# hongsukchoi/Pose2Mesh_RELEASE

Hardware: AMD Instinct MI355X
Metric: SMPL meshes/sec fwd+bwd at batch 256 (higher is better)
Workload: dtype f32 (emulated on the BF16 matrix pipe: every operand as 3 exact bf16 slices = 24-bit significands, 6 slice products per fp32 product, fp32 accumulate)

## Files before the change

pose2mesh_release_amd/csrc/basis.hip:

```cpp
#include <cstdlib>

#include "p2m_common.h"

namespace p2m {

constexpr int ROWS_PER_BLOCK = 4;

static int basis_spb() { return 8; }

static bool basis_tiled() {
  static int v = [] { const char* e = getenv("P2M_BASIS_TILED"); return e ? atoi(e) : 1; }();
  return v != 0;
}

__device__ __forceinline__ int xcd_swizzle(int bid, int nb) {
  return (nb & 7) == 0 ? (bid & 7) * (nb >> 3) + (bid >> 3) : bid;
}

__device__ __forceinline__ void fma4(float4& acc, float s, const float4& x) {
  acc.x = fmaf(s, x.x, acc.x); acc.y = fmaf(s, x.y, acc.y);
  acc.z = fmaf(s, x.z, acc.z); acc.w = fmaf(s, x.w, acc.w);
}

template <int LPR>
// ... 287 lines not shown
    const int u = q % U, sl = q / U, b = b0 + sl;
    if (b < B) {
      const float* src = G + ((long)b * V + pl.ucol[u0 + u]) * NC;
#pragma unroll
      for (int c = 0; c < NC; c++) xs[sl][u][c] = src[c];
    }
  }
  __syncthreads();
  const int i = t % TILE_RMAX, sl = t / TILE_RMAX, b = b0 + sl;
  if (i >= R || b >= B) return;
  const long ridx = (long)b * V + real_ids[r0 + i];
  float t1[NC], t2[NC];
#pragma unroll
  for (int c = 0; c < NC; c++) t1[c] = t2[c] = 0.f;
  for (int j = rowoff[i]; j < rowoff[i + 1]; j++) {
    const float4 en = ents[j];
    const float* q = xs[sl][__float_as_int(en.z)];
#pragma unroll
    for (int c = 0; c < NC; c++) {
      t1[c] = fmaf(en.x, q[c], t1[c]);
      t2[c] = fmaf(en.y, q[c], t2[c]);
    }
  }
  float* e = E + ridx * lde;
#pragma unroll
  for (int c = 0; c < NC; c++) {
    e[c] = G[ridx * NC + c];
    e[NC + c] = t1[c];
    e[2 * NC + c] = t2[c];
  }
  for (int c = 3 * NC; c < lde; c++) e[c] = 0.f;
}

}

using namespace p2m;

static int combine_small_launch(p2m_graph_t gh, const float* P, int32_t ldp, int32_t nc, const float* bias, float* Y,
                                int32_t B, int real_only, const int32_t* out_index, int32_t out_rows, float scale,
                                void* stream) {
  const Graph& g = *reinterpret_cast<const Graph*>(gh);
  const int* ids = real_only ? g.real_ids : nullptr;
  const int nset = real_only ? g.n_real : g.V;
  const long tot = (long)B * nset;
  if (tot == 0) return P2M_OK;
  hipStream_t s = (hipStream_t)stream;
  int skip_real = 0;
  const TilePlan& pl = g.plan[0];
  if (pl.ntiles > 0 && basis_tiled() && nc == 3) {
    hipLaunchKernelGGL(k_combine_small_tile<3>, dim3(pl.ntiles * cdiv(B, SMALL_SPB)), dim3(256), 0, s, pl, g.real_ids, g.V,
                       P, ldp, bias, Y, B, out_index, out_rows, scale);
    if (real_only) return check_launch("cheb_combine_small(tiled)");
    skip_real = 1;
  }
#define P2M_COMBINE(NCv) hipLaunchKernelGGL(k_combine_small<NCv>, dim3(cdiv(tot, 256)), dim3(256), 0, s, g, P, ldp, bias, \
                                            Y, B, ids, nset, out_index, out_rows, scale, skip_real)
  switch (nc) {
    case 1: P2M_COMBINE(1); break;
    case 2: P2M_COMBINE(2); break;
    case 3: P2M_COMBINE(3); break;
    case 4: P2M_COMBINE(4); break;
    default: set_error("p2m_cheb_combine_small: nc must be 1..4 (got %d)", nc); return P2M_ERR_INVALID;
  }
#undef P2M_COMBINE
  return check_launch("cheb_combine_small");
}

extern "C" int p2m_cheb_combine_small(p2m_graph_t gh, const float* P, int32_t ldp, int32_t nc, const float* bias,
                                      float* Y, int32_t B, void* stream) {
  P2M_CHECK_ARG(gh && P && Y && ldp >= 3 * nc, "null pointer or ldp < 3*nc");
  if (B <= 0) return P2M_OK;
  return combine_small_launch(gh, P, ldp, nc, bias, Y, B, 0, nullptr, 0, 1.f, stream);
}

extern "C" int p2m_cheb_combine_small_real(p2m_graph_t gh, const float* P, int32_t ldp, int32_t nc, const float* bias,
                                           float* Y, int32_t B, const int32_t* out_index, int32_t out_rows,
                                           float scale, void* stream) {
  P2M_CHECK_ARG(gh && P && Y && ldp >= 3 * nc, "null pointer or ldp < 3*nc");
  P2M_CHECK_ARG(out_index == nullptr || out_rows > 0, "out_rows must be positive with out_index");
  if (B <= 0) return P2M_OK;
  return combine_small_launch(gh, P, ldp, nc, bias, Y, B, 1, out_index, out_rows, scale, stream);
}

extern "C" int p2m_cheb_expand_small(p2m_graph_t gh, const float* G, int32_t nc, float* E, int32_t lde, int32_t B,
                                     void* stream) {
  P2M_CHECK_ARG(gh && G && E && lde >= 3 * nc, "null pointer or lde < 3*nc");
  if (B <= 0) return P2M_OK;
  const Graph& g = *reinterpret_cast<const Graph*>(gh);
  const long tot = (long)B * g.V;
  hipStream_t s = (hipStream_t)stream;
  int skip_real = 0;
  const TilePlan& pl = g.plan[0];
  if (pl.ntiles > 0 && basis_tiled() && nc == 3) {
    hipLaunchKernelGGL(k_expand_small_tile<3>, dim3(pl.ntiles * cdiv(B, SMALL_SPB)), dim3(256), 0, s, pl, g.real_ids, g.V,
                       G, E, lde, B);
    skip_real = 1;
  }
  switch (nc) {
    case 1: hipLaunchKernelGGL(k_expand_small<1>, dim3(cdiv(tot, 256)), dim3(256), 0, s, g, G, E, lde, B, skip_real); break;
    case 2: hipLaunchKernelGGL(k_expand_small<2>, dim3(cdiv(tot, 256)), dim3(256), 0, s, g, G, E, lde, B, skip_real); break;
    case 3: hipLaunchKernelGGL(k_expand_small<3>, dim3(cdiv(tot, 256)), dim3(256), 0, s, g, G, E, lde, B, skip_real); break;
    case 4: hipLaunchKernelGGL(k_expand_small<4>, dim3(cdiv(tot, 256)), dim3(256), 0, s, g, G, E, lde, B, skip_real); break;
    default: set_error("p2m_cheb_expand_small: nc must be 1..4 (got %d)", nc); return P2M_ERR_INVALID;
  }
  return check_launch("cheb_expand_small");
}


namespace p2m {
typedef float f32x4v __attribute__((ext_vector_type(4)));

template <int LPR>
__global__ __launch_bounds__(512, 2) void k_basis_tile(TilePlan pl, const float* __restrict__ X,
                                                        float* __restrict__ T1, float* __restrict__ T2, int B, int F,
                                                        long x_rows, int nset, int spb,
                                                        const float* __restrict__ in_scale = nullptr,
                                                        const float* __restrict__ in_shift = nullptr) {
  constexpr int NT = 512;
  constexpr int FB = LPR * 4;
  constexpr int RPI = NT / LPR;
  constexpr int NPF = (TILE_UCAP + RPI - 1) / RPI;
  __shared__ __attribute__((aligned(16))) float xs[TILE_UCAP * FB];
  __shared__ __attribute__((aligned(16))) f32x4v ents[TILE_ECAP];
  __shared__ int rowoff[TILE_RMAX + 1];

  const int lid = xcd_swizzle(blockIdx.x, gridDim.x);
  const int nsg = (B + spb - 1) / spb;
  if (lid >= pl.ntiles * nsg * (F / FB)) return;
  const int tile = lid % pl.ntiles;
// ... 195 lines not shown
```

pose2mesh_release_amd/csrc/bn.hip:

```cpp
#include <map>
#include <mutex>
#include <utility>

#include "p2m_common.h"

namespace p2m {

constexpr int FIN_COLS = 32;
constexpr int FIN_RG = 8;
constexpr int FIN_SPLITS = 48;
constexpr int FIN_SPLITS_MAX = 192;
static inline int fin_splits(long nrows) {
  return nrows >= 16384 ? FIN_SPLITS_MAX : (nrows >= 4096 ? 96 : FIN_SPLITS);
}
constexpr int FIN_Q = 4;
__device__ __forceinline__ void fin_sum(const double* __restrict__ part, int nsplits, int N, int n, bool live, double& t1,
                                        double& t2) {
  __shared__ double q1[FIN_Q][64], q2[FIN_Q][64];
  const int col = threadIdx.x & 63, q = threadIdx.x >> 6;
  const int per = nsplits / FIN_Q;
  t1 = 0.0;
  t2 = 0.0;
  if (live)
  for (int sp0 = q * per; sp0 < (q + 1) * per; sp0 += 12) {
// ... 342 lines not shown
    const float4 v = *reinterpret_cast<const float4*>(yb + (long)ids[i] * N + f);
    float d;
    d = v.x - mean.x; m2.x = fmaf(wv * d, d, m2.x);
    d = v.y - mean.y; m2.y = fmaf(wv * d, d, m2.y);
    d = v.z - mean.z; m2.z = fmaf(wv * d, d, m2.z);
    d = v.w - mean.w; m2.w = fmaf(wv * d, d, m2.w);
  }
  *reinterpret_cast<float4*>(&red[t * 4]) = m2;
  __syncthreads();
  if (rg == 0) {
    float4 a = make_float4(0.f, 0.f, 0.f, 0.f);
    for (int q = 0; q < RP; q++) {
      const float4 p = *reinterpret_cast<const float4*>(&red[(q * LPR + t) * 4]);
      a.x += p.x; a.y += p.y; a.z += p.z; a.w += p.w;
    }
    *reinterpret_cast<float4*>(st + (long)blockIdx.x * 2 * N + f) = tot;
    *reinterpret_cast<float4*>(st + (long)blockIdx.x * 2 * N + N + f) = a;
  }
}

__global__ __launch_bounds__(256) void k_class_reduce(const float* __restrict__ in, const float* __restrict__ w,
                                                       float* __restrict__ out, long M, int V, int F) {
  const long idx = (long)blockIdx.x * 256 + threadIdx.x;
  if (idx >= M * F) return;
  const long r = idx / F;
  const int f = (int)(idx - r * F);
  const int v = (int)(r % V);
  const int m = (int)w[v];
  float s = 0.f;
  for (int k = 0; k < m; k++) s += in[(r + k) * F + f];
  out[idx] = s;
}

constexpr int BWD_ROWS_PER_BLOCK = 512;
static inline int bwd_rows_per_block(long M) {
  if (M >= (long)BWD_ROWS_PER_BLOCK * 4096) return BWD_ROWS_PER_BLOCK;
  long r = (M + 4095) / 4096;
  r = (r + 63) / 64 * 64;
  return (int)(r < 64 ? 64 : r);
}

template <int LPR>
__global__ __launch_bounds__(256) void k_bn_bwd_reduce(const float* __restrict__ gx, const float* __restrict__ y,
                                                        const float* __restrict__ scale, const float* __restrict__ shift,
                                                        const float* __restrict__ mean, const float* __restrict__ invstd,
                                                        int relu, float* __restrict__ part, long M, RowMap m,
                                                        int rows_per_block) {
  constexpr int F = LPR * 4;
  constexpr int RP = 256 / LPR;
  __shared__ float red[2][RP][F];
  const int t = threadIdx.x;
  const int rloc = t / LPR, f = (t % LPR) * 4;
  const float4 sc = *reinterpret_cast<const float4*>(scale + f);
  const float4 sh = *reinterpret_cast<const float4*>(shift + f);
  const float4 mu = *reinterpret_cast<const float4*>(mean + f);
  const float4 is = *reinterpret_cast<const float4*>(invstd + f);
  float4 s0 = make_float4(0.f, 0.f, 0.f, 0.f), s1 = s0;
  const long r0 = (long)blockIdx.x * rows_per_block;
  long r1 = r0 + rows_per_block;
  if (r1 > M) r1 = M;
  const bool mapped = m.ids != nullptr;
  RowPos pb = {0u, 0u};
  if (mapped && r0 + rloc < r1) pb = row_pos(r0 + rloc, m);
  for (long rb = r0 + rloc; rb < r1; rb += 4 * RP) {
    float4 gq[4], vq[4];
#pragma unroll
// ... 693 lines not shown
  const int grid = cdiv(Mlog, APPLY_ROWS_PER_BLOCK);
  switch (F) {
    case 32:  hipLaunchKernelGGL(k_bn_bwd_apply<8>,  dim3(grid), dim3(256), 0, s, gx, y, scale, shift, mean, invstd, gamma, coef, relu, gy, Mlog, m, amax); break;
    case 64:  hipLaunchKernelGGL(k_bn_bwd_apply<16>, dim3(grid), dim3(256), 0, s, gx, y, scale, shift, mean, invstd, gamma, coef, relu, gy, Mlog, m, amax); break;
    case 128: hipLaunchKernelGGL(k_bn_bwd_apply<32>, dim3(grid), dim3(256), 0, s, gx, y, scale, shift, mean, invstd, gamma, coef, relu, gy, Mlog, m, amax); break;
    case 256: hipLaunchKernelGGL(k_bn_bwd_apply<64>, dim3(grid), dim3(256), 0, s, gx, y, scale, shift, mean, invstd, gamma, coef, relu, gy, Mlog, m, amax); break;
    default:
      hipLaunchKernelGGL(k_bn_bwd_apply_generic, dim3(cdiv(Mlog * F, 256)), dim3(256), 0, s, gx, y, scale, shift, mean, invstd, gamma, coef, relu, gy, Mlog, F, m, amax);
  }
  return check_launch("bn_bwd_apply");
}

extern "C" int p2m_stats_rows_w(p2m_graph_t gh, const float* y, int32_t B, int32_t N, float* stats, void* stream) {
  P2M_CHECK_ARG(gh && y && stats && N > 0, "null pointer or empty shape");
  const Graph& g = *reinterpret_cast<const Graph*>(gh);
  P2M_CHECK_ARG(g.w != nullptr, "the handle has no classes (p2m_graph_set_classes)");
  if (B <= 0 || g.n_fake == 0) return P2M_OK;
  const int tps = cdiv(g.n_fake, 128);
  if (N % 4 == 0 && N / 4 <= 256 && 256 % (N / 4) == 0)
    hipLaunchKernelGGL(k_stats_rows_w4, dim3(B * tps), dim3(256), 0, (hipStream_t)stream, y, g.fake_ids, g.fake_wts,
                       g.n_fake, g.V, tps, N, stats);
  else
    hipLaunchKernelGGL(k_stats_rows_w, dim3(B * tps), dim3(256), 0, (hipStream_t)stream, y, g.fake_ids, g.fake_wts,
                       g.n_fake, g.V, tps, N, stats);
  return check_launch("stats_rows_w");
}

extern "C" int p2m_class_reduce(p2m_graph_t gh, const float* in, float* out, int32_t B, int32_t F, void* stream) {
  P2M_CHECK_ARG(gh && in && out && F > 0, "null pointer or empty shape");
  const Graph& g = *reinterpret_cast<const Graph*>(gh);
  P2M_CHECK_ARG(g.w != nullptr, "the handle has no classes (p2m_graph_set_classes)");
  if (B <= 0) return P2M_OK;
  const long M = (long)B * g.V;
  hipLaunchKernelGGL(k_class_reduce, dim3(cdiv(M * F, 256)), dim3(256), 0, (hipStream_t)stream, in, g.w, out, M, g.V, F);
  return check_launch("class_reduce");
}

extern "C" int p2m_pair_sum(const float* in, float* out, int64_t Mout, int32_t F, p2m_graph_t classes, void* stream) {
  P2M_CHECK_ARG(in && out && F > 0 && F % 4 == 0, "null pointer or feature width not a multiple of 4");
  if (Mout <= 0) return P2M_OK;
  const float* w;
  int V;
  P2M_CHECK_ARG(class_table(classes, 2 * Mout, &w, &V) && (w == nullptr || V % 2 == 0),
                "row count is not a multiple of the level's (even) vertex count");
  long tot = Mout * (F / 4);
  hipLaunchKernelGGL(k_pair_sum, dim3(cdiv(tot, 256)), dim3(256), 0, (hipStream_t)stream, in, out, (long)Mout, F, w, V);
  return check_launch("pair_sum");
}

extern "C" int p2m_lerp_bwd_add(const float* g, float* dst, int64_t M, int32_t F, int32_t Fres, void* stream) {
  P2M_CHECK_ARG(g && dst && F > 0 && Fres > 0, "null pointer or empty shape");
  if (M <= 0) return P2M_OK;
  if (Fres == 2 * F && F % 2 == 0) {
    hipLaunchKernelGGL(k_lerp_bwd_add_half, dim3(cdiv(M * (F / 2), 256)), dim3(256), 0, (hipStream_t)stream, g, dst,
                       (long)M, F);
    return check_launch("lerp_bwd_add");
  }
  long tot = M * Fres;
  hipLaunchKernelGGL(k_lerp_bwd_add, dim3(cdiv(tot, 256)), dim3(256), 0, (hipStream_t)stream, g, dst, (long)M, F, Fres);
  return check_launch("lerp_bwd_add");
}
```

pose2mesh_release_amd/csrc/capi.hip:

```cpp
#include <algorithm>
#include <cmath>
#include <cstdarg>
#include <cstdlib>
#include <map>
#include <utility>
#include <vector>

#include "p2m_common.h"

namespace p2m {

static thread_local char g_err[512] = "";

void set_error(const char* fmt, ...) {
  va_list ap;
  va_start(ap, fmt);
  vsnprintf(g_err, sizeof(g_err), fmt, ap);
  va_end(ap);
}

int check_launch(const char* what) {
  hipError_t e = hipGetLastError();
  if (e != hipSuccess) {
    set_error("%s: HIP launch failed: %s", what, hipGetErrorString(e));
    return P2M_ERR_HIP;
  }
  return P2M_OK;
}

static int upload(const void* src, size_t bytes, void** dst) {
  hipError_t e = hipMalloc(dst, bytes ? bytes : 4);
  if (e != hipSuccess) {
    set_error("hipMalloc(%zu) failed: %s", bytes, hipGetErrorString(e));
    return P2M_ERR_NOMEM;
  }
  if (bytes) {
    e = hipMemcpy(*dst, src, bytes, hipMemcpyHostToDevice);
    if (e != hipSuccess) {
      set_error("hipMemcpy H2D failed: %s", hipGetErrorString(e));
      return P2M_ERR_HIP;
    }
  }
  return P2M_OK;
}

struct FlatRows {
  std::vector<int> rp{0}, src;
  std::vector<float> a, b;
  void push(int s, float x, float y) { src.push_back(s); a.push_back(x); b.push_back(y); }
  void end_row() { rp.push_back((int)src.size()); }
  int n() const { return (int)rp.size() - 1; }
};

static inline unsigned short f16_bits(float v) {
  const _Float16 h = (_Float16)v;
  unsigned short b;
  memcpy(&b, &h, sizeof(b));
  return b;
}

// ... 504 lines not shown
```

pose2mesh_release_amd/csrc/gemm.hip:

```cpp
#include <cstdlib>
#include <type_traits>

#include "p2m_split.h"

namespace p2m {

constexpr int BM = 128;
constexpr int BK = 32;
constexpr int AS_LD = BK + 1;

struct GemmArgs {
  const float* A[3];
  const float* Bm;
  const float* bias;
  const float* addend;
  const float* act_scale;
  const float* act_shift;
  int act_relu;
  int pair_out;
  float* C[3];
  float* stats;
  long M;
  int nplanesA, Ka, a0_shift;
  int N, Nc;
// ... 1748 lines not shown
      const _Float16 h = (_Float16)y;
      const _Float16 l = (_Float16)(y - (float)h);
      dst[0] = __builtin_bit_cast(unsigned short, h);
      dst[sl] = __builtin_bit_cast(unsigned short, l);
    }
  }
}

template <int NS>
__global__ __launch_bounds__(256) void k_conv_weights_images(const ConvWeights* __restrict__ d) {
  const ConvWeights c = d[blockIdx.y];
  const float* __restrict__ W = c.W;
  const int Fout = c.Fout, Fin = c.Fin, ld = 3 * c.Fin;
  const float a = c.fake_a, b = c.fake_b;
  const unsigned word = NS == 2 ? *c.amax : 0u;
  write_weight_image<NS>(c.Bx_f, 3 * Fin, Fout, word, 0, [&](int k, int n) {
    const int kk = k / Fin, fin = k - kk * Fin;
    return W[(long)n * ld + fin * 3 + kk];
  });
  write_weight_image<NS>(c.Bx_ef, Fin, Fout, word, c.eff_bits, [&](int k, int n) {
    const float* w = W + (long)n * ld + k * 3;
    return w[0] + a * w[1] + b * w[2];
  });
  write_weight_image<NS>(c.Bx_b, 3 * Fout, Fin, word, 0, [&](int k, int n) {
    const int kk = k / Fout, fo = k - kk * Fout;
    return W[(long)fo * ld + n * 3 + kk];
  });
  write_weight_image<NS>(c.Bx_eb, Fout, Fin, word, c.eff_bits, [&](int k, int n) {
    const float* w = W + (long)k * ld + n * 3;
    return w[0] + a * w[1] + b * w[2];
  });
}

constexpr int UNP_CG = 8;
__global__ __launch_bounds__(32 * UNP_CG) void k_weight_grad_unpack(
    const float* __restrict__ P, const float* __restrict__ Pdb, int nchunks, float* __restrict__ dW,
    float* __restrict__ db, int Fout, int Fin, int K, int accumulate, int layout, int pdb_stride,
    const float* __restrict__ P2, const float* __restrict__ Pdb2, int nchunks2, float fake_a, float fake_b) {
  __shared__ double red[UNP_CG][32];
  const int e = threadIdx.x & 31, cg = threadIdx.x >> 5;
  const long idx = (long)blockIdx.x * 32 + e;
  const long tot = (long)Fout * Fin * K;
  int fout = 0, k = 0, fin = 0;
  double s = 0.0;
  if (idx < tot) {
    if (layout == 0) {
      fout = (int)(idx % Fout);
      long kk = idx / Fout;
      k = (int)(kk / Fin); fin = (int)(kk % Fin);
    } else if (layout == 2) {
      fout = (int)(idx / Fin);
      fin = (int)(idx - (long)fout * Fin);
    } else {
      long nn = idx % ((long)K * Fout);
      fin = (int)(idx / ((long)K * Fout));
      k = (int)(nn / Fout); fout = (int)(nn % Fout);
    }
    float t0 = 0.f, t1 = 0.f, t2 = 0.f, t3 = 0.f;
    int c = cg;
    for (; c + 3 * UNP_CG < nchunks; c += 4 * UNP_CG) {
      t0 += P[(long)c * tot + idx];
      t1 += P[(long)(c + UNP_CG) * tot + idx];
      t2 += P[(long)(c + 2 * UNP_CG) * tot + idx];
      t3 += P[(long)(c + 3 * UNP_CG) * tot + idx];
    }
    for (; c < nchunks; c += UNP_CG) t0 += P[(long)c * tot + idx];
// ... 58 lines not shown
}

extern "C" int p2m_weight_split(const float* Bm, int32_t K, int32_t N, int32_t arith, const void* amax_in,
                                int32_t amax_bits, void* Bx, void* stream) {
  P2M_CHECK_ARG(Bm && Bx && K > 0 && N > 0, "null pointer or empty shape");
  P2M_CHECK_ARG(K % 16 == 0, "K must be a multiple of 16");
  P2M_CHECK_ARG(arith == P2M_ARITH_BF16X3 || arith == P2M_ARITH_F16X2, "arith must be P2M_ARITH_BF16X3 or P2M_ARITH_F16X2");
  const int Npad = cdiv(N, 128) * 128;
  const dim3 grid(cdiv((long)Npad * K, 256));
  unsigned short* bx = static_cast<unsigned short*>(Bx);
  if (arith == P2M_ARITH_F16X2) {
    const unsigned* word = static_cast<const unsigned*>(amax_in);
    P2M_CHECK_ARG(amax_bits >= 0 && amax_bits <= 30, "amax_bits out of range");
    if (word == nullptr) {
      unsigned* trailer = const_cast<unsigned*>(weight_amax_word(Bx, arith, Npad, K));
      hipLaunchKernelGGL(k_amax_one_block, dim3(1), dim3(1024), 0, (hipStream_t)stream, Bm, (long)K * N, trailer);
      word = trailer;
      amax_bits = 0;
    }
    hipLaunchKernelGGL(k_weight_split<2>, grid, dim3(256), 0, (hipStream_t)stream, Bm, bx, K, N, Npad, word, amax_bits);
  } else {
    hipLaunchKernelGGL(k_weight_split<3>, grid, dim3(256), 0, (hipStream_t)stream, Bm, bx, K, N, Npad, nullptr, 0);
  }
  return check_launch("weight_split");
}

extern "C" int p2m_conv_weights_prepare(const p2m_conv_weights* dev_desc, int32_t n, int32_t arith, void* stream) {
  static_assert(sizeof(p2m_conv_weights) == sizeof(ConvWeights), "descriptor layout");
  P2M_CHECK_ARG(dev_desc != nullptr && n > 0, "null descriptor array or no layers");
  P2M_CHECK_ARG(arith == P2M_ARITH_BF16X3 || arith == P2M_ARITH_F16X2, "arith must be P2M_ARITH_BF16X3 or P2M_ARITH_F16X2");
  const ConvWeights* d = reinterpret_cast<const ConvWeights*>(dev_desc);
  hipStream_t s = (hipStream_t)stream;
  const dim3 grid(96, n);
  if (arith == P2M_ARITH_F16X2) {
    hipLaunchKernelGGL(k_conv_weights_amax, dim3(n), dim3(1024), 0, s, d);
    hipLaunchKernelGGL(k_conv_weights_images<2>, grid, dim3(256), 0, s, d);
  } else {
    hipLaunchKernelGGL(k_conv_weights_images<3>, grid, dim3(256), 0, s, d);
  }
  return check_launch("conv_weights_prepare");
}

extern "C" int p2m_amax(const float* x, int64_t n, void* word, void* stream) {
  P2M_CHECK_ARG(x && word && n >= 0, "null pointer");
  P2M_CHECK_ARG((reinterpret_cast<uintptr_t>(x) & 3) == 0, "x must be 4-byte aligned");
  if (n == 0) return P2M_OK;
  long head = (long)((16 - (reinterpret_cast<uintptr_t>(x) & 15)) & 15) / 4;
  if (head > n) head = n;
  const long n4 = (n - head) / 4;
  const int tail = (int)(n - head - 4 * n4);
  const int grid = (int)(n4 < 256l * 4 * 1024 ? (n4 > 0 ? cdiv(n4, 256 * 4) : 1) : 1024);
  hipLaunchKernelGGL(k_amax, dim3(grid), dim3(256), 0, (hipStream_t)stream, x, (int)head, n4, tail,
                     static_cast<unsigned*>(word));
  return check_launch("amax");
}

extern "C" int p2m_amax_rows(p2m_graph_t gh, int32_t row_set, const float* x, int32_t B, int32_t F, void* word,
                             void* stream) {
  P2M_CHECK_ARG(gh && x && word, "null pointer");
  P2M_CHECK_ARG(row_set >= 0 && row_set <= 4, "row_set must be 0 (live rows) or 1..4");
  P2M_CHECK_ARG(F > 0 && F % 4 == 0, "F must be a positive multiple of 4");
  const Graph& gr = *reinterpret_cast<const Graph*>(gh);
  RowSet rs;
  if (row_set == 0) {
    rs.V = gr.V;
    rs.ids = gr.live_ids;
    rs.n = gr.live_ids ? gr.n_live : gr.V;
  } else {
    rs = row_set_of(gr, row_set);
  }
  if (B <= 0 || rs.n == 0) return P2M_OK;
// ... 367 lines not shown
```

pose2mesh_release_amd/csrc/loss.hip:

```cpp
#include "p2m_common.h"

namespace p2m {

struct LossArgs {
  const float* cam;
  const int* perm;
  const float* gt_mesh;
  const float* valid_mesh;
  const int* faces;
  const int* vf_ptr;
  const int* vf_idx;
  const int* jr_ptr;
  const int* jr_idx;
  const float* jr_val;
  const int* vj_ptr;
  const int* vj_idx;
  const float* vj_val;
  const float* gt_pose;
  const float* valid_pose;
  float* face_grad;
  float* pose_sign;
  float* partial;
  float* grad_cam;
  int B, V0, nv, F, J, npart;
// ... 24 lines not shown
  if (threadIdx.x == 0)
    for (int i = 0; i < (int)(blockDim.x >> 6); i++) s += sh[i];
  __syncthreads();
  return s;
}

__global__ __launch_bounds__(256) void k_pose_regress(LossArgs a) {
  __shared__ float sh[4];
  const int idx = blockIdx.x * 256 + threadIdx.x;
  float loss = 0.f;
  if (idx < a.B * a.J) {
    const int b = idx / a.J, j = idx - b * a.J;
    const float* cam = a.cam + (long)b * a.V0 * 3;
    float s0 = 0.f, s1 = 0.f, s2 = 0.f;
    for (int k = a.jr_ptr[j]; k < a.jr_ptr[j + 1]; k++) {
      const float w = a.jr_val[k];
      const float* p = cam + (long)a.perm[a.jr_idx[k]] * 3;
      s0 = fmaf(w, p[0] * 1000.f, s0);
      s1 = fmaf(w, p[1] * 1000.f, s1);
      s2 = fmaf(w, p[2] * 1000.f, s2);
    }
    const float val = a.valid_pose ? a.valid_pose[idx] : 1.f;
    const float pose[3] = {s0, s1, s2};
    for (int c = 0; c < 3; c++) {
      const float d = val * pose[c] - val * a.gt_pose[(long)idx * 3 + c];
      loss += fabsf(d);
      a.pose_sign[(long)idx * 3 + c] = a.s_joint * val * sgn(d) * 1000.f;
    }
  }
  const float sl = block_sum(loss, sh);
  if (threadIdx.x == 0) a.partial[3 * a.npart + blockIdx.x] = sl * a.s_joint;
}

__global__ __launch_bounds__(256) void k_face_terms(LossArgs a) {
  __shared__ float sh[4];
  const long idx = (long)blockIdx.x * 256 + threadIdx.x;
  float l_normal = 0.f, l_edge = 0.f;
  if (idx < (long)a.B * a.F) {
    const int b = (int)(idx / a.F), f = (int)(idx % a.F);
    const int i0 = a.faces[f * 3], i1 = a.faces[f * 3 + 1], i2 = a.faces[f * 3 + 2];
    const float* cam = a.cam + (long)b * a.V0 * 3;
    const float* gt = a.gt_mesh + (long)b * a.nv * 3;
    const V3 p0 = ld3(cam + (long)a.perm[i0] * 3), p1 = ld3(cam + (long)a.perm[i1] * 3), p2 = ld3(cam + (long)a.perm[i2] * 3);
    const V3 g0 = ld3(gt + (long)i0 * 3), g1 = ld3(gt + (long)i1 * 3), g2 = ld3(gt + (long)i2 * 3);
    float n1, n2, n3;
    const V3 e1 = normalize(sub(p1, p0), &n1), e2 = normalize(sub(p2, p0), &n2), e3 = normalize(sub(p2, p1), &n3);
    const V3 ng = normalize(cross(normalize(sub(g1, g0)), normalize(sub(g2, g0))));
    const float c1 = dot(e1, ng), c2 = dot(e2, ng), c3 = dot(e3, ng);
    l_normal = fabsf(c1) + fabsf(c2) + fabsf(c3);
    const V3 q1 = scale(sub(ng, scale(e1, c1)), a.s_normal * sgn(c1) / fmaxf(n1, 1e-12f));
    const V3 q2 = scale(sub(ng, scale(e2, c2)), a.s_normal * sgn(c2) / fmaxf(n2, 1e-12f));
    const V3 q3 = scale(sub(ng, scale(e3, c3)), a.s_normal * sgn(c3) / fmaxf(n3, 1e-12f));
    V3 d0 = scale(add(q1, q2), -1.f);
    V3 d1 = sub(q1, q3);
    V3 d2 = add(q2, q3);
    if (a.s_normal == 0.f) d0 = d1 = d2 = V3{0.f, 0.f, 0.f};
    const V3 u01 = sub(p0, p1), u02 = sub(p0, p2), u12 = sub(p1, p2);
    const float o1 = sqrtf(dot(u01, u01)), o2 = sqrtf(dot(u02, u02)), o3 = sqrtf(dot(u12, u12));
    const V3 h01 = sub(g0, g1), h02 = sub(g0, g2), h12 = sub(g1, g2);
    const float t1 = sqrtf(dot(h01, h01)), t2 = sqrtf(dot(h02, h02)), t3 = sqrtf(dot(h12, h12));
    l_edge = fabsf(o1 - t1) + fabsf(o2 - t2) + fabsf(o3 - t3);
    if (a.s_edge != 0.f) {
      const V3 r1 = scale(u01, a.s_edge * sgn(o1 - t1) / o1);
      const V3 r2 = scale(u02, a.s_edge * sgn(o2 - t2) / o2);
      const V3 r3 = scale(u12, a.s_edge * sgn(o3 - t3) / o3);
      d0 = add(d0, add(r1, r2));
      d1 = add(d1, sub(r3, r1));
      d2 = sub(d2, add(r2, r3));
    }
    float* fg = a.face_grad + idx * 9;
    fg[0] = d0.x; fg[1] = d0.y; fg[2] = d0.z;
    fg[3] = d1.x; fg[4] = d1.y; fg[5] = d1.z;
    fg[6] = d2.x; fg[7] = d2.y; fg[8] = d2.z;
  }
  const float sn = block_sum(l_normal, sh);
  const float se = block_sum(l_edge, sh);
  if (threadIdx.x == 0) {
    a.partial[1 * a.npart + blockIdx.x] = sn * a.s_normal;
    a.partial[2 * a.npart + blockIdx.x] = se * a.s_edge;
  }
}

__global__ __launch_bounds__(256) void k_vertex_grad(LossArgs a) {
  __shared__ float sh[4];
  const long idx = (long)blockIdx.x * 256 + threadIdx.x;
  float l_v = 0.f;
  if (idx < (long)a.B * a.nv) {
    const int b = (int)(idx / a.nv), v = (int)(idx % a.nv);
    const float val = a.valid_mesh ? a.valid_mesh[idx] : 1.f;
    const float* p = a.cam + ((long)b * a.V0 + a.perm[v]) * 3;
    const float* g = a.gt_mesh + idx * 3;
    float gr[3];
    for (int c = 0; c < 3; c++) {
      const float d = val * p[c] - val * g[c];
      l_v += fabsf(d);
      gr[c] = a.s_vertex * val * sgn(d);
    }
    const float* fgb = a.face_grad + (long)b * a.F * 9;
    for (int k = a.vf_ptr[v]; k < a.vf_ptr[v + 1]; k++) {
      const float* fg = fgb + (long)a.vf_idx[k] * 3;
      gr[0] += fg[0]; gr[1] += fg[1]; gr[2] += fg[2];
    }
    const float* ps = a.pose_sign + (long)b * a.J * 3;
    for (int k = a.vj_ptr[v]; k < a.vj_ptr[v + 1]; k++) {
      const float w = a.vj_val[k];
      const int j = a.vj_idx[k];
      gr[0] = fmaf(w, ps[j * 3], gr[0]);
      gr[1] = fmaf(w, ps[j * 3 + 1], gr[1]);
      gr[2] = fmaf(w, ps[j * 3 + 2], gr[2]);
    }
    if (a.grad_cam) {
      float* o = a.grad_cam + ((long)b * a.V0 + a.perm[v]) * 3;
      o[0] = gr[0]; o[1] = gr[1]; o[2] = gr[2];
    }
  }
  const float sv = block_sum(l_v, sh);
  if (threadIdx.x == 0) a.partial[0 * a.npart + blockIdx.x] = sv * a.s_vertex;
}

__global__ __launch_bounds__(256) void k_loss_finalize(const float* __restrict__ partial, int npart, int n0, int n1, int n2, int n3,
                                float* __restrict__ losses) {
  const int which = blockIdx.x;
  const int n = which == 0 ? n0 : which == 1 ? n1 : which == 2 ? n2 : n3;
  __shared__ double wsum[4];
  double s0 = 0.0, s1 = 0.0, s2 = 0.0, s3 = 0.0;
  const float* pp = partial + (long)which * npart;
  int i = threadIdx.x;
  for (; i + 768 < n; i += 1024) {
    s0 += (double)pp[i];
    s1 += (double)pp[i + 256];
    s2 += (double)pp[i + 512];
    s3 += (double)pp[i + 768];
  }
  for (; i < n; i += 256) s0 += (double)pp[i];
  double s = (s0 + s1) + (s2 + s3);
  for (int o = 32; o > 0; o >>= 1) s += __shfl_xor(s, o);
  if ((threadIdx.x & 63) == 0) wsum[threadIdx.x >> 6] = s;
  __syncthreads();
  if (threadIdx.x == 0) losses[which] = (float)((wsum[0] + wsum[1]) + (wsum[2] + wsum[3]));
}

__global__ __launch_bounds__(1024) void k_coord_loss(const float* __restrict__ pred, const float* __restrict__ target,
                                                     const float* __restrict__ valid, int per_mask, long n, float w,
                                                     float* __restrict__ loss, float* __restrict__ grad) {
  __shared__ double wsum[16];
  double s = 0.0;
  const float gscale = w / (float)n;
  for (long i = threadIdx.x; i < n; i += 1024) {
    const float v = valid ? valid[i / per_mask] : 1.f;
    const float d = pred[i] * v - target[i] * v;
// ... 72 lines not shown
                             const int32_t* vf_idx, const int32_t* jr_ptr, const int32_t* jr_idx, const float* jr_val,
                             const int32_t* vj_ptr, const int32_t* vj_idx, const float* vj_val, int32_t J,
                             const float* gt_pose, const float* valid_pose, float w_vertex, float w_normal,
                             float w_edge, float w_joint, float* workspace, float* losses, float* grad_cam, int32_t B,
                             void* stream) {
  P2M_CHECK_ARG(cam_mesh && perm && gt_mesh && faces && vf_ptr && vf_idx && gt_pose && workspace && losses,
                "null pointer");
  P2M_CHECK_ARG(jr_ptr && jr_idx && jr_val && vj_ptr && vj_idx && vj_val, "null joint-regressor CSR/CSC");
  P2M_CHECK_ARG(B > 0 && V0 > 0 && nv > 0 && F > 0 && J > 0, "empty shape");
  LossArgs a;
  a.cam = cam_mesh; a.perm = perm; a.gt_mesh = gt_mesh; a.valid_mesh = valid_mesh; a.faces = faces;
  a.vf_ptr = vf_ptr; a.vf_idx = vf_idx; a.gt_pose = gt_pose; a.valid_pose = valid_pose;
  a.jr_ptr = jr_ptr; a.jr_idx = jr_idx; a.jr_val = jr_val; a.vj_ptr = vj_ptr; a.vj_idx = vj_idx; a.vj_val = vj_val;
  a.B = B; a.V0 = V0; a.nv = nv; a.F = F; a.J = J;
  const int nb_face = cdiv((long)B * F, 256), nb_vert = cdiv((long)B * nv, 256), nb_pose = cdiv((long)B * J, 256);
  a.npart = (int)loss_nparts(B, nv, F, J);
  a.face_grad = workspace;
  a.pose_sign = workspace + (long)B * F * 9;
  a.partial = a.pose_sign + (long)B * J * 3;
  a.grad_cam = grad_cam;
  a.s_vertex = w_vertex / ((float)B * nv * 3);
  a.s_normal = w_normal / ((float)B * F * 3);
  a.s_edge = w_edge / ((float)B * F * 3);
  a.s_joint = w_joint / ((float)B * J * 3);
  hipStream_t s = (hipStream_t)stream;
  if (grad_cam) {
    hipError_t e = hipMemsetAsync(grad_cam, 0, sizeof(float) * (size_t)B * V0 * 3, s);
    if (e != hipSuccess) {
      set_error("p2m_mesh_loss: memset failed: %s", hipGetErrorString(e));
      return P2M_ERR_HIP;
    }
  }
  hipLaunchKernelGGL(k_pose_regress, dim3(nb_pose), dim3(256), 0, s, a);
  hipLaunchKernelGGL(k_face_terms, dim3(nb_face), dim3(256), 0, s, a);
  hipLaunchKernelGGL(k_vertex_grad, dim3(nb_vert), dim3(256), 0, s, a);
  hipLaunchKernelGGL(k_loss_finalize, dim3(4), dim3(256), 0, s, a.partial, a.npart, nb_vert, nb_face, nb_face, nb_pose, losses);
  return check_launch("mesh_loss");
}

extern "C" int p2m_coord_loss(const float* pred, const float* target, const float* valid, int32_t per_mask, int64_t n,
                              float w, float* loss, float* grad, void* stream) {
  P2M_CHECK_ARG(pred && target && loss && n > 0 && per_mask > 0, "null pointer or empty shape");
  hipLaunchKernelGGL(k_coord_loss, dim3(1), dim3(1024), 0, (hipStream_t)stream, pred, target, valid, per_mask, (long)n, w,
                     loss, grad);
  return check_launch("coord_loss");
}
```

pose2mesh_release_amd/csrc/p2m_common.h:

```cpp
#pragma once
#include <hip/hip_runtime.h>
#include <cstdint>
#include <cstdio>
#include <cstring>

#include "../../include/p2m.h"

namespace p2m {

void set_error(const char* fmt, ...);
int check_launch(const char* what);

struct TilePlan {
  int ntiles = 0;
  int* tile_row = nullptr;
  int* tile_u = nullptr;
  int* ucol = nullptr;
  int* erow = nullptr;
  float4* ent = nullptr;
  float* tile_cnt = nullptr;
  unsigned short* ltx = nullptr;
  int lt_exp = 0;
  unsigned short* ltx3 = nullptr;
};
constexpr int TILE_UPAD = 128;
constexpr int TILE_LTX_ELEMS = (TILE_UPAD / 16) * 2 * 64 * 16;
constexpr int TILE_LTX3_ELEMS = (TILE_UPAD / 16) * 3 * 64 * 16;
constexpr int TILE_RMAX = 32;
constexpr int TILE_UCAP = 120;
constexpr int TILE_ECAP = 896;

struct Graph {
  int V = 0;
  int nnz = 0;
  int nnz_L = 0;
  int max_row = 0;
  int plane_bits = 0;
  int* rowptr = nullptr;
  int* col = nullptr;
  float* a = nullptr;
  float* b = nullptr;
  int n_real = 0, n_fake = 0;
  int* real_ids = nullptr;
  int* fake_ids = nullptr;
// ... 5 lines not shown
  float* w = nullptr;
  int* rep_of = nullptr;
  float* fake_wts = nullptr;
  float* fake_tile_w = nullptr;
  int n_fake_all = 0;
  int* live_ids = nullptr;
  int n_live = 0;
  int* live_pairs = nullptr;
  int n_live_pairs = 0;
};

constexpr int ID_PREFETCH_STAGES = 5, ID_STAGE_ROWS = 16;
constexpr int ID_SLACK = ID_PREFETCH_STAGES * ID_STAGE_ROWS;

struct RowSet {
  const int* ids = nullptr;
  int n = 0;
  int V = 0;
};
static inline bool row_set_valid(int which) { return which >= 1 && which <= 4; }
static inline RowSet row_set_of(const Graph& g, int which) {
  RowSet r;
  r.V = which >= 3 ? g.V / 2 : g.V;
  if (which == 1) { r.ids = g.real_ids; r.n = g.n_real; }
  else if (which == 2) { r.ids = g.fake_ids; r.n = g.n_fake; }
  else if (which == 3) { r.ids = g.pair_real_ids; r.n = g.n_pair_real; }
  else { r.ids = g.pair_fake_ids; r.n = g.n_pair_fake; }
  return r;
}

static inline int cdiv(long a, long b) { return (int)((a + b - 1) / b); }
#ifdef __HIPCC__
__device__ __forceinline__ int cdiv_dev(int a, int b) { return (a + b - 1) / b; }
#endif

#ifdef __HIPCC__
__device__ __forceinline__ void amax_commit(unsigned* word, float m) {
#pragma unroll
  for (int o = 32; o > 0; o >>= 1) m = fmaxf(m, __shfl_xor(m, o));
  if ((threadIdx.x & 63) == 0 && m > 0.f) {
    const unsigned bits = __float_as_uint(m);
    if (bits > __hip_atomic_load(word, __ATOMIC_RELAXED, __HIP_MEMORY_SCOPE_AGENT)) atomicMax(word, bits);
  }
}
__device__ __forceinline__ float amax_abs(float v) {
  const float a = fabsf(v);
  return a < __builtin_inff() ? a : 0.f;
}
__device__ __forceinline__ float amax4(float m, const float* o) {
  return fmaxf(fmaxf(m, fmaxf(amax_abs(o[0]), amax_abs(o[1]))), fmaxf(amax_abs(o[2]), amax_abs(o[3])));
}
#endif

#define P2M_CHECK_ARG(cond, msg)                       \
  do {                                                 \
    if (!(cond)) {                                     \
      p2m::set_error("%s: %s", __func__, msg);         \
      return P2M_ERR_INVALID;                          \
    }                                                  \
  } while (0)

}
```

Measured before the change: 6599.

## Stage narrow 3-wide rows through shared memory for coalesced vector stores

Result: faster. 6672, median of 6 (+1.1%).

```diff
diff --git a/pose2mesh_release_amd/csrc/basis.hip b/pose2mesh_release_amd/csrc/basis.hip
--- a/pose2mesh_release_amd/csrc/basis.hip
+++ b/pose2mesh_release_amd/csrc/basis.hip
@@ -343,6 +343,112 @@
   for (int c = 3 * NC; c < lde; c++) e[c] = 0.f;
 }
 
+constexpr int EXP_NC = 3, EXP_Q = 3;
+
+__device__ __forceinline__ void expand_stage_row(float4* r, const float* g, const float* t1, const float* t2) {
+  r[0] = make_float4(g[0], g[1], g[2], t1[0]);
+  r[1] = make_float4(t1[1], t1[2], t2[0], t2[1]);
+  r[2] = make_float4(t2[2], 0.f, 0.f, 0.f);
+}
+
+__device__ __forceinline__ void expand_copy_out(const float4* res, const long* erow, int nrows, float* __restrict__ E, int lde) {
+  const int L4 = lde >> 2;
+  for (int u = threadIdx.x; u < nrows * L4; u += 256) {
+    const int i = u / L4, q = u - i * L4;
+    const long er = erow[i];
+    if (er < 0) continue;
+    const float4 v = q < EXP_Q ? res[i * EXP_Q + q] : make_float4(0.f, 0.f, 0.f, 0.f);
+    reinterpret_cast<float4*>(E + er * lde)[q] = v;
+  }
+}
+
+__global__ __launch_bounds__(256) void k_expand_small_rows(Graph g, const float* __restrict__ G, float* __restrict__ E,
+                                                            int lde, int B, int skip_real) {
+  __shared__ float4 res[256 * EXP_Q];
+  __shared__ long erow[256];
+  const long idx = (long)blockIdx.x * 256 + threadIdx.x;
+  long er = -1;
+  if (idx < (long)B * g.V) {
+    const int row = (int)(idx % g.V);
+    const int j0 = g.rowptr[row], j1 = g.rowptr[row + 1];
+    const bool live = !(skip_real && j1 - j0 > 1) && !(g.w != nullptr && g.w[row] == 0.f);
+    if (live) {
+      const long base = (idx - row) * EXP_NC;
+      float t1[EXP_NC], t2[EXP_NC], gv[EXP_NC];
+#pragma unroll
+      for (int c = 0; c < EXP_NC; c++) t1[c] = t2[c] = 0.f;
+      for (int j = j0; j < j1; j++) {
+        const float* q = G + base + (long)g.col[j] * EXP_NC;
+        const float a = g.a[j], b = g.b[j];
+#pragma unroll
+        for (int c = 0; c < EXP_NC; c++) {
+          t1[c] = fmaf(a, q[c], t1[c]);
+          t2[c] = fmaf(b, q[c], t2[c]);
+        }
+      }
+#pragma unroll
+      for (int c = 0; c < EXP_NC; c++) gv[c] = G[idx * EXP_NC + c];
+      expand_stage_row(res + threadIdx.x * EXP_Q, gv, t1, t2);
+      er = idx;
+    }
+  }
+  erow[threadIdx.x] = er;
+  __syncthreads();
+  expand_copy_out(res, erow, 256, E, lde);
+}
+
+__global__ __launch_bounds__(256) void k_expand_small_tile_rows(TilePlan pl, const int* __restrict__ real_ids, int V,
+                                                                 const float* __restrict__ G, float* __restrict__ E, int lde,
+                                                                 int B) {
+  __shared__ float4 ents[TILE_ECAP];
+  __shared__ int rowoff[TILE_RMAX + 1];
+  __shared__ float xs[SMALL_SPB][TILE_UCAP][EXP_NC];
+  __shared__ float4 res[256 * EXP_Q];
+  __shared__ long erow[256];
+  const int bid = xcd_block_id(blockIdx.x, gridDim.x);
+  const int tile = bid % pl.ntiles, sg = bid / pl.ntiles;
+  const int t = threadIdx.x;
+  const int r0 = pl.tile_row[tile], R = pl.tile_row[tile + 1] - r0;
+  const int u0 = pl.tile_u[tile], U = pl.tile_u[tile + 1] - u0;
+  const int e0 = pl.erow[r0], nE = pl.erow[r0 + R] - e0;
+  for (int i = t; i < nE; i += 256) ents[i] = pl.ent[e0 + i];
+  if (t <= R) rowoff[t] = pl.erow[r0 + t] - e0;
+  const int b0 = sg * SMALL_SPB;
+  for (int q = t; q < U * SMALL_SPB; q += 256) {
+    const int u = q % U, sl = q / U, b = b0 + sl;
+    if (b < B) {
+      const float* src = G + ((long)b * V + pl.ucol[u0 + u]) * EXP_NC;
+#pragma unroll
+      for (int c = 0; c < EXP_NC; c++) xs[sl][u][c] = src[c];
+    }
+  }
+  __syncthreads();
+  const int i = t % TILE_RMAX, sl = t / TILE_RMAX, b = b0 + sl;
+  long er = -1;
+  if (i < R && b < B) {
+    const long ridx = (long)b * V + real_ids[r0 + i];
+    float t1[EXP_NC], t2[EXP_NC], gv[EXP_NC];
+#pragma unroll
+    for (int c = 0; c < EXP_NC; c++) t1[c] = t2[c] = 0.f;
+    for (int j = rowoff[i]; j < rowoff[i + 1]; j++) {
+      const float4 en = ents[j];
+      const float* q = xs[sl][__float_as_int(en.z)];
+#pragma unroll
+      for (int c = 0; c < EXP_NC; c++) {
+        t1[c] = fmaf(en.x, q[c], t1[c]);
+        t2[c] = fmaf(en.y, q[c], t2[c]);
+      }
+    }
+#pragma unroll
+    for (int c = 0; c < EXP_NC; c++) gv[c] = G[ridx * EXP_NC + c];
+    expand_stage_row(res + t * EXP_Q, gv, t1, t2);
+    er = ridx;
+  }
+  erow[t] = er;
+  __syncthreads();
+  expand_copy_out(res, erow, 256, E, lde);
+}
+
 }
 
 using namespace p2m;
@@ -402,10 +508,19 @@
   hipStream_t s = (hipStream_t)stream;
   int skip_real = 0;
   const TilePlan& pl = g.plan[0];
+  const bool rows16 = nc == 3 && lde % 4 == 0 && (reinterpret_cast<uintptr_t>(E) & 15) == 0 && narrow_rows();
   if (pl.ntiles > 0 && basis_tiled() && nc == 3) {
-    hipLaunchKernelGGL(k_expand_small_tile<3>, dim3(pl.ntiles * cdiv(B, SMALL_SPB)), dim3(256), 0, s, pl, g.real_ids, g.V,
-                       G, E, lde, B);
+    if (rows16)
+      hipLaunchKernelGGL(k_expand_small_tile_rows, dim3(pl.ntiles * cdiv(B, SMALL_SPB)), dim3(256), 0, s, pl, g.real_ids,
+                         g.V, G, E, lde, B);
+    else
+      hipLaunchKernelGGL(k_expand_small_tile<3>, dim3(pl.ntiles * cdiv(B, SMALL_SPB)), dim3(256), 0, s, pl, g.real_ids, g.V,
+                         G, E, lde, B);
     skip_real = 1;
+  }
+  if (rows16) {
+    hipLaunchKernelGGL(k_expand_small_rows, dim3(cdiv(tot, 256)), dim3(256), 0, s, g, G, E, lde, B, skip_real);
+    return check_launch("cheb_expand_small");
   }
   switch (nc) {
     case 1: hipLaunchKernelGGL(k_expand_small<1>, dim3(cdiv(tot, 256)), dim3(256), 0, s, g, G, E, lde, B, skip_real); break;
diff --git a/pose2mesh_release_amd/csrc/bn.hip b/pose2mesh_release_amd/csrc/bn.hip
--- a/pose2mesh_release_amd/csrc/bn.hip
+++ b/pose2mesh_release_amd/csrc/bn.hip
@@ -398,6 +398,39 @@
   out[idx] = s;
 }
 
+constexpr int CR3_ROWS = 1024;
+__global__ __launch_bounds__(256) void k_class_reduce3(const float* __restrict__ in, const float* __restrict__ w,
+                                                        float* __restrict__ out, long M, int V) {
+  __shared__ float4 buf4[CR3_ROWS * 3 / 4];
+  float* buf = reinterpret_cast<float*>(buf4);
+  const int t = threadIdx.x;
+  const long r0 = (long)blockIdx.x * CR3_ROWS;
+  const int rows = (int)(M - r0 < CR3_ROWS ? M - r0 : CR3_ROWS);
+  const int n = rows * 3, n4 = n >> 2;
+  const float* src = in + r0 * 3;
+  float* dst = out + r0 * 3;
+  for (int i = t; i < n4; i += 256) buf4[i] = reinterpret_cast<const float4*>(src)[i];
+  if (t < n - 4 * n4) buf[4 * n4 + t] = src[4 * n4 + t];
+  __syncthreads();
+  const int v0 = (int)(r0 % V);
+  for (int row = t; row < rows; row += 256) {
+    const int m = (int)w[(v0 + row) % V];
+    float s0 = 0.f, s1 = 0.f, s2 = 0.f;
+    if (m > 0) {
+      s0 += buf[3 * row]; s1 += buf[3 * row + 1]; s2 += buf[3 * row + 2];
+      const float* p = src + 3 * row;
+      for (int k = 1; k < m; k++) {
+        p += 3;
+        s0 += p[0]; s1 += p[1]; s2 += p[2];
+      }
+    }
+    buf[3 * row] = s0; buf[3 * row + 1] = s1; buf[3 * row + 2] = s2;
+  }
+  __syncthreads();
+  for (int i = t; i < n4; i += 256) reinterpret_cast<float4*>(dst)[i] = buf4[i];
+  if (t < n - 4 * n4) dst[4 * n4 + t] = buf[4 * n4 + t];
+}
+
 constexpr int BWD_ROWS_PER_BLOCK = 512;
 static inline int bwd_rows_per_block(long M) {
   if (M >= (long)BWD_ROWS_PER_BLOCK * 4096) return BWD_ROWS_PER_BLOCK;
@@ -1157,7 +1190,11 @@
   P2M_CHECK_ARG(g.w != nullptr, "the handle has no classes (p2m_graph_set_classes)");
   if (B <= 0) return P2M_OK;
   const long M = (long)B * g.V;
-  hipLaunchKernelGGL(k_class_reduce, dim3(cdiv(M * F, 256)), dim3(256), 0, (hipStream_t)stream, in, g.w, out, M, g.V, F);
+  const bool aligned = ((reinterpret_cast<uintptr_t>(in) | reinterpret_cast<uintptr_t>(out)) & 15) == 0;
+  if (F == 3 && aligned && narrow_rows())
+    hipLaunchKernelGGL(k_class_reduce3, dim3(cdiv(M, CR3_ROWS)), dim3(256), 0, (hipStream_t)stream, in, g.w, out, M, g.V);
+  else
+    hipLaunchKernelGGL(k_class_reduce, dim3(cdiv(M * F, 256)), dim3(256), 0, (hipStream_t)stream, in, g.w, out, M, g.V, F);
   return check_launch("class_reduce");
 }
 
diff --git a/pose2mesh_release_amd/csrc/capi.hip b/pose2mesh_release_amd/csrc/capi.hip
--- a/pose2mesh_release_amd/csrc/capi.hip
+++ b/pose2mesh_release_amd/csrc/capi.hip
@@ -26,6 +26,11 @@
     return P2M_ERR_HIP;
   }
   return P2M_OK;
+}
+
+bool narrow_rows() {
+  static const bool v = [] { const char* e = getenv("P2M_NARROW_ROWS"); return e ? atoi(e) != 0 : true; }();
+  return v;
 }
 
 static int upload(const void* src, size_t bytes, void** dst) {
diff --git a/pose2mesh_release_amd/csrc/gemm.hip b/pose2mesh_release_amd/csrc/gemm.hip
--- a/pose2mesh_release_amd/csrc/gemm.hip
+++ b/pose2mesh_release_amd/csrc/gemm.hip
@@ -1804,6 +1804,144 @@
   });
 }
 
+constexpr int WI_T = 32;
+constexpr int WI_LD = 3 * WI_T + 1;
+
+__device__ __forceinline__ float weight_eff_value(const float* w, float a, float b) { return w[0] + a * w[1] + b * w[2]; }
+
+template <int NS>
+__device__ __forceinline__ void store_k8(unsigned short* __restrict__ dst, long sl, const float (&v)[8], float sc) {
+  unsigned short s[NS][8];
+#pragma unroll
+  for (int e = 0; e < 8; e++) {
+    if constexpr (NS == 3) {
+      unsigned h, m, l;
+      split3(v[e], h, m, l);
+      s[0][e] = (unsigned short)(h >> 16);
+      s[1][e] = (unsigned short)(m >> 16);
+      s[2][e] = (unsigned short)(l >> 16);
+    } else {
+      const float y = v[e] * sc;
+      const _Float16 h = (_Float16)y;
+      const _Float16 l = (_Float16)(y - (float)h);
+      s[0][e] = __builtin_bit_cast(unsigned short, h);
+      s[1][e] = __builtin_bit_cast(unsigned short, l);
+    }
+  }
+#pragma unroll
+  for (int q = 0; q < NS; q++) {
+    u32x4 p;
+#pragma unroll
+    for (int i = 0; i < 4; i++) p[i] = (unsigned)s[q][2 * i] | ((unsigned)s[q][2 * i + 1] << 16);
+    *reinterpret_cast<u32x4*>(dst + q * sl) = p;
+  }
+}
+
+template <int NS>
+__device__ __forceinline__ float weight_image_scale(unsigned short* Bx, int K, int Npad, unsigned word, int bits) {
+  if constexpr (NS == 2) {
+    if (blockIdx.x == 0 && threadIdx.x == 0)
+      *reinterpret_cast<unsigned*>(Bx + (long)NS * Npad * K) =
+          word == 0u ? 0u : __float_as_uint(__builtin_ldexpf(__uint_as_float(word), bits));
+    return exp2_int(slice_scale_exp(word, bits));
+  }
+  return 1.f;
+}
+
+template <int NS>
+__global__ __launch_bounds__(256) void k_conv_weights_images_tiled(const ConvWeights* __restrict__ d) {
+  __shared__ float tile[WI_T][WI_LD];
+  const ConvWeights c = d[blockIdx.y];
+  const float* __restrict__ W = c.W;
+  const int Fout = c.Fout, Fin = c.Fin, ld = 3 * c.Fin;
+  const float a = c.fake_a, b = c.fake_b;
+  const unsigned word = NS == 2 ? *c.amax : 0u;
+  const int t = threadIdx.x;
+  const auto tiled = [](const unsigned short* Bx, int kdim) {
+    return Bx != nullptr && kdim % 16 == 0 && (reinterpret_cast<uintptr_t>(Bx) & 15) == 0;
+  };
+  const bool tf = tiled(c.Bx_f, Fin), tef = tiled(c.Bx_ef, Fin), tb = tiled(c.Bx_b, Fout), teb = tiled(c.Bx_eb, Fout);
+  if (!tf)
+    write_weight_image<NS>(c.Bx_f, 3 * Fin, Fout, word, 0, [&](int k, int n) {
+      const int kk = k / Fin, fin = k - kk * Fin;
+      return W[(long)n * ld + fin * 3 + kk];
+    });
+  if (!tef)
+    write_weight_image<NS>(c.Bx_ef, Fin, Fout, word, c.eff_bits, [&](int k, int n) {
+      return weight_eff_value(W + (long)n * ld + k * 3, a, b);
+    });
+  if (!tb)
+    write_weight_image<NS>(c.Bx_b, 3 * Fout, Fin, word, 0, [&](int k, int n) {
+      const int kk = k / Fout, fo = k - kk * Fout;
+      return W[(long)fo * ld + n * 3 + kk];
+    });
+  if (!teb)
+    write_weight_image<NS>(c.Bx_eb, Fout, Fin, word, c.eff_bits, [&](int k, int n) {
+      return weight_eff_value(W + (long)k * ld + n * 3, a, b);
+    });
+  if (!(tf || tef || tb || teb)) return;
+  const int FoP = cdiv_dev(Fout, 128) * 128, FiP = cdiv_dev(Fin, 128) * 128;
+  const long sl_o = (long)FoP * 16, sl_i = (long)FiP * 16;
+  float sc_f = 1.f, sc_ef = 1.f, sc_b = 1.f, sc_eb = 1.f;
+  if (tf) sc_f = weight_image_scale<NS>(c.Bx_f, 3 * Fin, FoP, word, 0);
+  if (tef) sc_ef = weight_image_scale<NS>(c.Bx_ef, Fin, FoP, word, c.eff_bits);
+  if (tb) sc_b = weight_image_scale<NS>(c.Bx_b, 3 * Fout, FiP, word, 0);
+  if (teb) sc_eb = weight_image_scale<NS>(c.Bx_eb, Fout, FiP, word, c.eff_bits);
+  const int nti = FiP / WI_T, nt = (FoP / WI_T) * nti;
+  for (int tl = blockIdx.x; tl < nt; tl += gridDim.x) {
+    const int fo0 = (tl / nti) * WI_T, fin0 = (tl - (tl / nti) * nti) * WI_T;
+    const bool has_o = fo0 < Fout, has_i = fin0 < Fin;
+    if (!has_o && !has_i) continue;
+    __syncthreads();
+    for (int e = t; e < WI_T * 3 * WI_T; e += 256) {
+      const int r = e / (3 * WI_T), cc = e - r * (3 * WI_T);
+      const int fo = fo0 + r, col = 3 * fin0 + cc;
+      tile[r][cc] = (fo < Fout && col < ld) ? W[(long)fo * ld + col] : 0.f;
+    }
+    __syncthreads();
+    if (has_i && (tf || tef)) {
+      for (int j = t; j < 64 * 2 * 4; j += 256) {
+        const int half = j & 1, nl = (j >> 1) & 31, g = (j >> 6) & 1, kk = j >> 7;
+        const int fl = 16 * g + 8 * half, fin = fin0 + fl, n = fo0 + nl;
+        if (fin >= Fin) continue;
+        float v[8];
+        if (kk < 3) {
+          if (!tf) continue;
+#pragma unroll
+          for (int e = 0; e < 8; e++) v[e] = n < Fout ? tile[nl][(fl + e) * 3 + kk] : 0.f;
+          const int k = kk * Fin + fin;
+          store_k8<NS>(c.Bx_f + (long)(k >> 4) * NS * sl_o + (long)n * 16 + (k & 15), sl_o, v, sc_f);
+        } else {
+          if (!tef) continue;
+#pragma unroll
+          for (int e = 0; e < 8; e++) v[e] = n < Fout ? weight_eff_value(&tile[nl][(fl + e) * 3], a, b) : 0.f;
+          store_k8<NS>(c.Bx_ef + (long)(fin >> 4) * NS * sl_o + (long)n * 16 + (fin & 15), sl_o, v, sc_ef);
+        }
+      }
+    }
+    if (has_o && (tb || teb)) {
+      for (int j = t; j < 64 * 2 * 4; j += 256) {
+        const int half = j & 1, nl = (j >> 1) & 31, g = (j >> 6) & 1, kk = j >> 7;
+        const int rl = 16 * g + 8 * half, fo = fo0 + rl, n = fin0 + nl;
+        if (fo >= Fout) continue;
+        float v[8];
+        if (kk < 3) {
+          if (!tb) continue;
+#pragma unroll
+          for (int e = 0; e < 8; e++) v[e] = n < Fin ? tile[rl + e][nl * 3 + kk] : 0.f;
+          const int k = kk * Fout + fo;
+          store_k8<NS>(c.Bx_b + (long)(k >> 4) * NS * sl_i + (long)n * 16 + (k & 15), sl_i, v, sc_b);
+        } else {
+          if (!teb) continue;
+#pragma unroll
+          for (int e = 0; e < 8; e++) v[e] = n < Fin ? weight_eff_value(&tile[rl + e][nl * 3], a, b) : 0.f;
+          store_k8<NS>(c.Bx_eb + (long)(fo >> 4) * NS * sl_i + (long)n * 16 + (fo & 15), sl_i, v, sc_eb);
+        }
+      }
+    }
+  }
+}
+
 constexpr int UNP_CG = 8;
 __global__ __launch_bounds__(32 * UNP_CG) void k_weight_grad_unpack(
     const float* __restrict__ P, const float* __restrict__ Pdb, int nchunks, float* __restrict__ dW,
@@ -1928,11 +2066,14 @@
   const ConvWeights* d = reinterpret_cast<const ConvWeights*>(dev_desc);
   hipStream_t s = (hipStream_t)stream;
   const dim3 grid(96, n);
+  const bool tiled = narrow_rows();
   if (arith == P2M_ARITH_F16X2) {
     hipLaunchKernelGGL(k_conv_weights_amax, dim3(n), dim3(1024), 0, s, d);
-    hipLaunchKernelGGL(k_conv_weights_images<2>, grid, dim3(256), 0, s, d);
+    if (tiled) hipLaunchKernelGGL(k_conv_weights_images_tiled<2>, grid, dim3(256), 0, s, d);
+    else hipLaunchKernelGGL(k_conv_weights_images<2>, grid, dim3(256), 0, s, d);
   } else {
-    hipLaunchKernelGGL(k_conv_weights_images<3>, grid, dim3(256), 0, s, d);
+    if (tiled) hipLaunchKernelGGL(k_conv_weights_images_tiled<3>, grid, dim3(256), 0, s, d);
+    else hipLaunchKernelGGL(k_conv_weights_images<3>, grid, dim3(256), 0, s, d);
   }
   return check_launch("conv_weights_prepare");
 }
diff --git a/pose2mesh_release_amd/csrc/loss.hip b/pose2mesh_release_amd/csrc/loss.hip
--- a/pose2mesh_release_amd/csrc/loss.hip
+++ b/pose2mesh_release_amd/csrc/loss.hip
@@ -80,9 +80,17 @@
   if (threadIdx.x == 0) a.partial[3 * a.npart + blockIdx.x] = sl * a.s_joint;
 }
 
+template <bool XCD>
+__device__ __forceinline__ int loss_block_id() {
+  if constexpr (XCD) return xcd_block_id(blockIdx.x, gridDim.x);
+  else return blockIdx.x;
+}
+
+template <bool XCD>
 __global__ __launch_bounds__(256) void k_face_terms(LossArgs a) {
   __shared__ float sh[4];
-  const long idx = (long)blockIdx.x * 256 + threadIdx.x;
+  const int bid = loss_block_id<XCD>();
+  const long idx = (long)bid * 256 + threadIdx.x;
   float l_normal = 0.f, l_edge = 0.f;
   if (idx < (long)a.B * a.F) {
     const int b = (int)(idx / a.F), f = (int)(idx % a.F);
@@ -124,14 +132,16 @@
   const float sn = block_sum(l_normal, sh);
   const float se = block_sum(l_edge, sh);
   if (threadIdx.x == 0) {
-    a.partial[1 * a.npart + blockIdx.x] = sn * a.s_normal;
-    a.partial[2 * a.npart + blockIdx.x] = se * a.s_edge;
-  }
-}
-
+    a.partial[1 * a.npart + bid] = sn * a.s_normal;
+    a.partial[2 * a.npart + bid] = se * a.s_edge;
+  }
+}
+
+template <bool XCD>
 __global__ __launch_bounds__(256) void k_vertex_grad(LossArgs a) {
   __shared__ float sh[4];
-  const long idx = (long)blockIdx.x * 256 + threadIdx.x;
+  const int bid = loss_block_id<XCD>();
+  const long idx = (long)bid * 256 + threadIdx.x;
   float l_v = 0.f;
   if (idx < (long)a.B * a.nv) {
     const int b = (int)(idx / a.nv), v = (int)(idx % a.nv);
@@ -163,7 +173,7 @@
     }
   }
   const float sv = block_sum(l_v, sh);
-  if (threadIdx.x == 0) a.partial[0 * a.npart + blockIdx.x] = sv * a.s_vertex;
+  if (threadIdx.x == 0) a.partial[0 * a.npart + bid] = sv * a.s_vertex;
 }
 
 __global__ __launch_bounds__(256) void k_loss_finalize(const float* __restrict__ partial, int npart, int n0, int n1, int n2, int n3,
@@ -302,8 +312,13 @@
     }
   }
   hipLaunchKernelGGL(k_pose_regress, dim3(nb_pose), dim3(256), 0, s, a);
-  hipLaunchKernelGGL(k_face_terms, dim3(nb_face), dim3(256), 0, s, a);
-  hipLaunchKernelGGL(k_vertex_grad, dim3(nb_vert), dim3(256), 0, s, a);
+  if (narrow_rows()) {
+    hipLaunchKernelGGL(k_face_terms<true>, dim3(nb_face), dim3(256), 0, s, a);
+    hipLaunchKernelGGL(k_vertex_grad<true>, dim3(nb_vert), dim3(256), 0, s, a);
+  } else {
+    hipLaunchKernelGGL(k_face_terms<false>, dim3(nb_face), dim3(256), 0, s, a);
+    hipLaunchKernelGGL(k_vertex_grad<false>, dim3(nb_vert), dim3(256), 0, s, a);
+  }
   hipLaunchKernelGGL(k_loss_finalize, dim3(4), dim3(256), 0, s, a.partial, a.npart, nb_vert, nb_face, nb_face, nb_pose, losses);
   return check_launch("mesh_loss");
 }
diff --git a/pose2mesh_release_amd/csrc/p2m_common.h b/pose2mesh_release_amd/csrc/p2m_common.h
--- a/pose2mesh_release_amd/csrc/p2m_common.h
+++ b/pose2mesh_release_amd/csrc/p2m_common.h
@@ -10,6 +10,7 @@
 
 void set_error(const char* fmt, ...);
 int check_launch(const char* what);
+bool narrow_rows();
 
 struct TilePlan {
   int ntiles = 0;
@@ -81,6 +82,10 @@
 static inline int cdiv(long a, long b) { return (int)((a + b - 1) / b); }
 #ifdef __HIPCC__
 __device__ __forceinline__ int cdiv_dev(int a, int b) { return (a + b - 1) / b; }
+__device__ __forceinline__ int xcd_block_id(int bid, int nb) {
+  const int x = bid & 7, q = nb >> 3, r = nb & 7;
+  return x * q + (x < r ? x : r) + (bid >> 3);
+}
 #endif
 
 #ifdef __HIPCC__
```
